# Allisterh/CCMMshadowrateVAR-code

Hardware: AMD Instinct MI355X
Metric: Gibbs sweeps/sec (chains x vintages) N=20 p=12 (higher is better)
Workload: dtype f64

## Files before the change

### ccmmshadowratevar-code_amd/csrc/ccmm_lag.h

```cpp
#pragma once
#include <algorithm>

#include "ccmm_internal.h"

namespace ccmm {

struct LagSel {
  const double* dpool;
  const int* idx;
  const int* colmap;
  int ldd, rows, p;
  int mode;
};
constexpr int kLagGramExport = 8;
constexpr int kLagNoSyrk = 1, kLagNoChol = 2;
constexpr int kLagNoFactorInv = 256;
constexpr int kLagNoTrailing = 1024;
constexpr int kLagNoV = 16, kLagNoXtv = 32, kLagNoSubst = 64, kLagNoXx = 128;

struct SolveXch {
  double* part;
  unsigned long long* flag;
  unsigned long long epoch;
};
constexpr int kSolveSplitMaxB = 64;

constexpr int kGlWaves = 8;
constexpr int kGlLd = 17;
constexpr int kGlTile = 16 * kGlLd;

__host__ __device__ constexpr int gl_ntile(int NT) { return NT * (NT + 1) / 2; }
__host__ __device__ constexpr int gl_tpw(int NT) { return (gl_ntile(NT) + kGlWaves - 1) / kGlWaves; }
__host__ __device__ constexpr int gl_tile(int NT, int i, int j) { return j * NT - j * (j - 1) / 2 + (i - j); }
__host__ __device__ constexpr int gl_tj(int NT, int g) {
  int tj = 0;
  while (tj < NT && g >= NT - tj) {
    g -= NT - tj;
    ++tj;
  }
  return tj;
}
__host__ __device__ constexpr int gl_ti(int NT, int g) {
  int tj = 0;
  while (tj < NT && g >= NT - tj) {
    g -= NT - tj;
    ++tj;
  }
  return tj + g;
}
__host__ __device__ constexpr int gl_out_len(int NT) { return gl_ntile(NT) * 256 + 256; }
inline size_t gl_lds_bytes(int NT, int rows, int ldd, int TP) {
  const size_t syrk = (size_t)rows * ldd + TP + 4;
  const size_t fac = 16 * NT + 8 + 64 + 2 * kGlTile + 2 * (size_t)NT * kGlTile + kGlWaves * kGlTile;
  return std::max(syrk, fac) * sizeof(double);
}

constexpr int kSlThreads = 512;

__host__ __device__ inline int sl_union(int NT, int TP) { return TP + 512; }
inline size_t sl_lds_bytes(int NT, int rows, int ldd, int TP, int nmax) {
  const size_t n = (size_t)rows * ldd + sl_union(NT, TP) + 256 + 256 + (size_t)nmax * nmax + 16;
  return n * sizeof(double) + (16 * NT + 32) * sizeof(int);
}

bool lag_supported_nt(int nt);
hipError_t lag_launch_gram(int NT, hipStream_t st, size_t lds, Dims d, const int* Tslot, LagSel ls,
                           ChainState cs, const double* iVdiag);
int lag_solve_resident(int NT, int nmax, size_t lds, int async);
hipError_t lag_launch_solve(int NT, int nmax, int async, hipStream_t st, size_t lds, Dims d, const int* Tslot,
                            const double* iVb, XSel xs, LagSel ls, ChainState cs, RngArgs ra, SolveXch xc);

}
```

### ccmmshadowratevar-code_amd/csrc/ccmm_lag.hip

```cpp
#include "ccmm_lag.h"

#include <cstdlib>

namespace ccmm {

struct GlArgs {
  const double* w;
  const double* iv;
  const int* colmap;
  double* out;
  int T, ldd, mode;
  const double* Dl;
  const double* swl;
};

__device__ __forceinline__ int gl_opaque(int v) {
  asm volatile("" : "+v"(v));
  return v;
}

__device__ __forceinline__ double gl_rsqrt_det(double d) { return rsqrt_det(d); }

__device__ __forceinline__ int gl_factor_inv(const double* Dg, double* Ws, int lane_in) {
  const int lane = gl_opaque(lane_in);
  double row[16];
  double rdiag = 1.0, dmin = 1.0;
#pragma unroll
  for (int m = 0; m < 16; ++m) row[m] = (lane < 16 && m <= lane) ? Dg[lane * kGlLd + m] : 0.0;
#pragma unroll
  for (int kk = 0; kk < 16; ++kk) {
    double dkk = readlane_d(row[kk], kk);
    dmin = fmin(dmin, dkk);
    const double rp = gl_rsqrt_det(fmax(dkk, 1e-300));
    if (lane == kk) rdiag = rp;
    const double lik = (lane > kk) ? row[kk] * rp : 0.0;
    row[kk] = lik;
#pragma unroll
    for (int m = kk + 1; m < 16; ++m) row[m] = fma(-lik, readlane_d(lik, m), row[m]);
  }
  const int bad = (dmin > 0.0) ? 0 : 1;
  const int c = lane;
  double x[16];
#pragma unroll
  for (int i = 0; i < 16; ++i) {
    double s0 = (i == c) ? 1.0 : 0.0, s1 = 0.0;
#pragma unroll
    for (int m = 0; m < i; m += 2) {
      s0 = fma(-readlane_d(row[m], i), x[m], s0);
      if (m + 1 < i) s1 = fma(-readlane_d(row[m + 1], i), x[m + 1], s1);
    }
    x[i] = (i >= c) ? (s0 + s1) * readlane_d(rdiag, i) : 0.0;
  }
  if (lane < 16) {
#pragma unroll
    for (int i = 0; i < 16; ++i) Ws[i * kGlLd + c] = x[i];
  }
  wave_lds_sync();
  return bad;
}

template <int NT, int W>
__device__ __forceinline__ void gl_syrk(const GlArgs& g, dbl4 (&acc)[gl_tpw(NT)], double& bs0, double& bs1,
                                        double& csum, int lane) {
  constexpr int NTILE = gl_ntile(NT);
  constexpr int TPW = gl_tpw(NT);
  const int lr = lane & 15, lq = lane >> 4;
#pragma unroll
  for (int k = 0; k < TPW; ++k) acc[k] = dbl4{0.0, 0.0, 0.0, 0.0};

  int off[NT];
#pragma unroll
  for (int b = 0; b < NT; ++b) off[b] = g.colmap[16 * b + lr];
  bs0 = 0.0;
  bs1 = 0.0;
  csum = 0.0;
  const int nks = (g.mode & kLagNoSyrk) ? 0 : (g.T + 3) >> 2;
  double raw[NT], sw = 0.0;
  auto load = [&](int ks) {
    const int t = 4 * ks + lq;
    sw = g.swl[t];
    const double* row = g.Dl + t * g.ldd;
#pragma unroll
    for (int b = 0; b < NT; ++b) raw[b] = row[off[b]];
  };
  if (nks > 0) load(0);
  for (int ks = 0; ks < nks; ++ks) {
    double frag[NT];
#pragma unroll
    for (int b = 0; b < NT; ++b) frag[b] = raw[b] * sw;
    const double swc = sw;
    load(ks + 1 < nks ? ks + 1 : ks);
    __builtin_amdgcn_sched_barrier(0);
#pragma unroll
    for (int k = 0; k < TPW; ++k) {
      if (W + kGlWaves * k < NTILE) {
        const int gi = W + kGlWaves * k;
        acc[k] = __builtin_amdgcn_mfma_f64_16x16x4f64(frag[gl_tj(NT, gi)], frag[gl_ti(NT, gi)], acc[k],
                                                      0, 0, 0);
      }
    }
    if (W < NT) bs0 = fma(frag[W < NT ? W : 0], swc, bs0);
    if (W + kGlWaves < NT) bs1 = fma(frag[W + kGlWaves < NT ? W + kGlWaves : 0], swc, bs1);
    csum = fma(swc, swc, csum);
    __builtin_amdgcn_sched_barrier(0);
  }
  bs0 += __shfl_xor(bs0, 16);
  bs0 += __shfl_xor(bs0, 32);
  bs1 += __shfl_xor(bs1, 16);
  bs1 += __shfl_xor(bs1, 32);
  csum += __shfl_xor(csum, 16);
  csum += __shfl_xor(csum, 32);
}

template <int NT>
__device__ __forceinline__ int gram_lag_factor(const GlArgs& g, double* sm, int tid, int W,
                                               dbl4 (&acc)[gl_tpw(NT)], double bs0, double bs1, double csum) {
  constexpr int NTILE = gl_ntile(NT);
  constexpr int TPW = gl_tpw(NT);
  constexpr int KL = 16 * NT;
  const int lane = tid & 63, lr0 = lane & 15, lq0 = lane >> 4;
  const int lr = lr0, lq = lq0;
  int bad = 0;
  int sti[TPW], stj[TPW];
#pragma unroll
  for (int k = 0; k < TPW; ++k) {
    const int gi = W + kGlWaves * k;
    sti[k] = gi < NTILE ? gl_ti(NT, gi) : 0;
    stj[k] = gi < NTILE ? gl_tj(NT, gi) : 0;
  }
  if (g.mode & kLagGramExport) {
    double* o = g.out;
#pragma unroll
    for (int k = 0; k < TPW; ++k) {
      const int gi = W + kGlWaves * k;
      if (gi < NTILE) {
#pragma unroll
        for (int r = 0; r < 4; ++r) o[gi * 256 + 64 * r + lane] = acc[k][r];
      }
    }
    if (lq == 0) {
      if (W < NT) o[NTILE * 256 + 1 + 16 * W + lr] = bs0;
      if (W + kGlWaves < NT) o[NTILE * 256 + 1 + 16 * (W + kGlWaves) + lr] = bs1;
    }
    if (W == 0 && lane == 0) o[NTILE * 256] = csum;
    return 0;
  }
  __syncthreads();

  double* lvec = sm;
  double* misc = lvec + KL;
  double* Dg = misc + 8;
  double* Pn0 = Dg + kGlTile;
  double* Ws = Pn0 + 2 * NT * kGlTile + W * kGlTile;

  if (lq == 0) {
    if (W < NT) lvec[16 * W + lr] = bs0;
    if (W + kGlWaves < NT) lvec[16 * (W + kGlWaves) + lr] = bs1;
  }
  if (W == 0 && lane == 0) misc[0] = csum;
  __syncthreads();
  const double G00 = misc[0] + g.iv[0];
  if (!(G00 > 0.0)) bad = 1;
  const double L00 = sqrt(G00 > 0.0 ? G00 : 1.0);
  const double rL00 = 1.0 / L00;
#pragma unroll
  for (int k = 0; k < TPW; ++k) {
    const int gi = W + kGlWaves * k;
    if (gi < NTILE) {
      const int ti = sti[k], tj = stj[k];
      const double lc = lvec[16 * ti + lr] * rL00;
#pragma unroll
      for (int r = 0; r < 4; ++r) {
        const int rowi = 16 * tj + lq + 4 * r;
        double v = fma(-(lvec[rowi] * rL00), lc, acc[k][r]);
        if (ti == tj && lq + 4 * r == lr) v += g.iv[1 + rowi];
        acc[k][r] = v;
      }
    }
  }
  __syncthreads();
  if (tid < KL) lvec[tid] *= rL00;
  __syncthreads();

  double* LinvB = Dg;
  const bool do_chol = !(g.mode & kLagNoChol);
  if (do_chol) {
    bool own = false;
#pragma unroll
    for (int k = 0; k < TPW; ++k) {
      const int gi = W + kGlWaves * k;
      if (gi < NTILE && sti[k] == 0 && stj[k] == 0) {
#pragma unroll
        for (int r = 0; r < 4; ++r) Ws[(lq + 4 * r) * kGlLd + lr] = acc[k][r];
        own = true;
      }
    }
    wave_lds_sync();
    if (own && !(g.mode & kLagNoFactorInv)) bad |= gl_factor_inv(Ws, LinvB, lane);
  }
  for (int p = 0; p < (do_chol ? NT : 0); ++p) {
    const int lr = gl_opaque(lr0), lq = gl_opaque(lq0);
    __syncthreads();
    double* Pn = Pn0;
#pragma unroll
    for (int k = 0; k < TPW; ++k) {
      const int gi = W + kGlWaves * k;
      if (gi < NTILE && stj[k] == p) {
        const int ti = sti[k];
        if (ti == p) {
#pragma unroll
          for (int r = 0; r < 4; ++r) acc[k][r] = LinvB[lr * kGlLd + lq + 4 * r];
        } else {
          dbl4 cc = dbl4{0.0, 0.0, 0.0, 0.0};
#pragma unroll
          for (int kk = 0; kk < 4; ++kk)
            cc = __builtin_amdgcn_mfma_f64_16x16x4f64(LinvB[lr * kGlLd + 4 * kk + lq], acc[k][kk], cc, 0, 0, 0);
#pragma unroll
          for (int r = 0; r < 4; ++r) Pn[ti * kGlTile + (lq + 4 * r) * kGlLd + lr] = cc[r];
          dbl4 mm = dbl4{0.0, 0.0, 0.0, 0.0};
#pragma unroll
          for (int kk = 0; kk < 4; ++kk)
            mm = __builtin_amdgcn_mfma_f64_16x16x4f64(LinvB[(4 * kk + lq) * kGlLd + lr], cc[kk], mm, 0, 0, 0);
          acc[k] = mm;
        }
      }
    }
    __syncthreads();
    if (p + 1 < NT && !(g.mode & kLagNoTrailing)) {
      const int q = p + 1;
      bool own = false;
#pragma unroll
      for (int k = 0; k < TPW; ++k) {
        const int gi = W + kGlWaves * k;
        if (gi < NTILE && sti[k] == q && stj[k] == q) {
#pragma unroll
          for (int kk = 0; kk < 4; ++kk) {
            const double pq = Pn[q * kGlTile + (4 * kk + lq) * kGlLd + lr];
            acc[k] = __builtin_amdgcn_mfma_f64_16x16x4f64(-pq, pq, acc[k], 0, 0, 0);
          }
#pragma unroll
          for (int r = 0; r < 4; ++r) Ws[(lq + 4 * r) * kGlLd + lr] = acc[k][r];
          own = true;
        }
      }
      wave_lds_sync();
      if (own && !(g.mode & kLagNoFactorInv)) bad |= gl_factor_inv(Ws, LinvB, lane);
#pragma unroll
      for (int k = 0; k < TPW; ++k) {
        const int gi = W + kGlWaves * k;
        if (gi < NTILE && stj[k] > p && !(sti[k] == q && stj[k] == q)) {
          const double* Pa = Pn + stj[k] * kGlTile + lq * kGlLd + lr;
          const double* Pb = Pn + sti[k] * kGlTile + lq * kGlLd + lr;
#pragma unroll
          for (int kk = 0; kk < 4; ++kk)
            acc[k] = __builtin_amdgcn_mfma_f64_16x16x4f64(-Pa[4 * kk * kGlLd], Pb[4 * kk * kGlLd], acc[k], 0, 0,
                                                          0);
        }
      }
    }
  }

  double* o = g.out;
  if (tid < KL) o[NTILE * 256 + 1 + tid] = lvec[tid];
  if (tid == 0) o[NTILE * 256] = rL00;
#pragma unroll
  for (int k = 0; k < TPW; ++k) {
    const int gi = W + kGlWaves * k;
    if (gi < NTILE) {
#pragma unroll
      for (int r = 0; r < 4; ++r) o[gi * 256 + 64 * r + lane] = acc[k][r];
    }
  }
  return bad;
}

template <int NT>
__global__ __launch_bounds__(512, 1) void k_gram_chol_lag(Dims d, const int* __restrict__ Tslot, LagSel ls,
                                                          ChainState cs, const double* __restrict__ iVdiag) {
  extern __shared__ double sm[];
  const int mat = blockIdx.x;
  const int c = mat / d.N, j = mat % d.N;
  const int s = cs.slot[c];
  const int tid = threadIdx.x;
  const int TP = d.TP;
  {
    const double* src = ls.dpool + (size_t)ls.idx[mat] * ls.rows * ls.ldd;
    const int n = ls.rows * ls.ldd;
    const double* w = cs.W + (size_t)mat * TP;
    double* swl = sm + n;
    int q = tid;
    for (; q < n; q += 32 * 512) {
      double v[32];
#pragma unroll
      for (int u = 0; u < 32; ++u) v[u] = (q + 512 * u < n) ? src[q + 512 * u] : 0.0;
      double wv[2];
#pragma unroll
      for (int u = 0; u < 2; ++u) wv[u] = (q == tid && tid + 512 * u < TP) ? w[tid + 512 * u] : 0.0;
#pragma unroll
      for (int u = 0; u < 32; ++u)
        if (q + 512 * u < n) sm[q + 512 * u] = v[u];
      if (q == tid) {
#pragma unroll
        for (int u = 0; u < 2; ++u)
          if (tid + 512 * u < TP + 4) swl[tid + 512 * u] = wv[u];
      }
    }
    for (int t = tid + 1024; t < TP + 4; t += 512) swl[t] = (t < TP) ? w[t] : 0.0;
  }
  __syncthreads();
  GlArgs g;
  g.T = Tslot[s];
  g.ldd = ls.ldd;
  g.mode = ls.mode;
  g.colmap = ls.colmap;
  g.iv = iVdiag + ((size_t)s * d.N + j) * d.KP;
  g.out = cs.G + (size_t)mat * d.KP * d.KP;
  g.Dl = sm;
  g.swl = sm + ls.rows * ls.ldd;
  g.w = nullptr;
  const int wave = __builtin_amdgcn_readfirstlane(tid >> 6);
  dbl4 acc[gl_tpw(NT)];
  double bs0, bs1, csum;
  switch (wave) {
    case 0: gl_syrk<NT, 0>(g, acc, bs0, bs1, csum, tid & 63); break;
    case 1: gl_syrk<NT, 1>(g, acc, bs0, bs1, csum, tid & 63); break;
    case 2: gl_syrk<NT, 2>(g, acc, bs0, bs1, csum, tid & 63); break;
    case 3: gl_syrk<NT, 3>(g, acc, bs0, bs1, csum, tid & 63); break;
    case 4: gl_syrk<NT, 4>(g, acc, bs0, bs1, csum, tid & 63); break;
    case 5: gl_syrk<NT, 5>(g, acc, bs0, bs1, csum, tid & 63); break;
    case 6: gl_syrk<NT, 6>(g, acc, bs0, bs1, csum, tid & 63); break;
    case 7: gl_syrk<NT, 7>(g, acc, bs0, bs1, csum, tid & 63); break;
    default: __builtin_unreachable();
  }
  const int bad = gram_lag_factor<NT>(g, sm, tid, wave, acc, bs0, bs1, csum);
  if (bad && (tid & 63) == 0) atomicOr(&cs.status[c], 2);
}

#ifdef CCMM_ABLATION
__device__ unsigned long long g_solve_prof[8];
extern "C" int ccmm_solve_prof(unsigned long long* out, int reset) {
  if (hipMemcpyFromSymbol(out, HIP_SYMBOL(g_solve_prof), sizeof(g_solve_prof)) != hipSuccess) return -1;
  if (reset) {
    static const unsigned long long z[8] = {};
    if (hipMemcpyToSymbol(HIP_SYMBOL(g_solve_prof), z, sizeof(z)) != hipSuccess) return -1;
  }
  return 0;
}
#define SL_CLK(x) const unsigned long long x = clock64()
#define SL_ACC(k, a, b) \
  if (c == 0 && blockIdx.y == 0 && tid == 0) atomicAdd(&g_solve_prof[k], (b) - (a))
#else
#define SL_CLK(x)
#define SL_ACC(k, a, b)
#endif
constexpr int kSlWaves = kSlThreads / 64;
template <int NT, int NMAX, bool RO>
__global__ __launch_bounds__(kSlThreads) void k_cta_solve_lag(Dims d, const int* __restrict__ Tslot,
                                                                const double* __restrict__ iVb, XSel xs, LagSel ls,
                                                                ChainState cs, RngArgs ra, SolveXch xc) {
  constexpr int NTILE = gl_ntile(NT);
  static_assert(kSlWaves == 8, "row-owned substitutions and the X'v t-halves: 8 waves");
  static_assert(!RO || NT == 1 || NT == 15, "row-owned substitutions: NT 1 or 15");
  constexpr int TPW = RO ? NT : (gl_ntile(NT) + kSlWaves - 1) / kSlWaves;
  constexpr int KL = 16 * NT;
  extern __shared__ double sm[];
  const int N = d.N, TP = d.TP, K = d.K, KP = d.KP;
  const int ldd = ls.ldd, rows = ls.rows;
  double* Dl = sm;
  double* vl = Dl + rows * ldd;
  double* part = vl + TP;
  double* rl = vl + sl_union(NT, TP);
  double* xl = rl + 256;
  double* Al = xl + 256;
  double* red = Al + NMAX * NMAX;
  int* cm = reinterpret_cast<int*>(red + 16);
  int* zdone = cm + KL;
  int* cnt = zdone + 16;
  const int c = blockIdx.x;
  const int s = cs.slot[c];
  const int T = Tslot[s];
  const int tid = threadIdx.x, lane0 = tid & 63;
  const int wave = __builtin_amdgcn_readfirstlane(tid >> 6);
  const Rng rng = ra.make(c);
  const bool split = gridDim.y > 1;
  const int hh = split ? (int)blockIdx.y : 0;
  const int th = (T + 1) >> 1;
  const int tlo = (split && hh) ? th : 0, thi = (split && !hh) ? th : TP;
  const double* ih2 = cs.ih2 + (size_t)c * N * TP;
  const double* Y = xs.ypool + (size_t)xs.yidx[c] * N * TP;
  double* E = cs.E + (size_t)c * N * TP;
  for (int q = tid; q < N * N; q += kSlThreads) Al[(q % N) + (q / N) * NMAX] = cs.A[(size_t)c * N * N + q];
  for (int q = tid; q < KL; q += kSlThreads) cm[q] = ls.colmap[q];
  int sti[TPW], stj[TPW];
  const int rHi = NT - 1 - wave, rLo = wave - 1;
  const bool hasHi = rHi >= 0, hasLo = wave >= 1 && rLo < rHi;
  const int nHi = hasHi ? rHi + 1 : 0, nLo = hasLo ? rLo + 1 : 0;
#pragma unroll
  for (int k = 0; k < TPW; ++k) {
    if constexpr (RO) {
      sti[k] = (k < nHi) ? rHi : rLo;
      stj[k] = (k < nHi) ? k : k - nHi;
    } else {
      const int gi = wave + kSlWaves * k;
      sti[k] = gi < NTILE ? gl_ti(NT, gi) : 0;
      stj[k] = gi < NTILE ? gl_tj(NT, gi) : 0;
    }
  }
  auto slot_of = [&](int k) -> int {
    if constexpr (RO) return (k < nHi + nLo) ? gl_tile(NT, sti[k], stj[k]) : -1;
    const int gi = wave + kSlWaves * k;
    return gi < NTILE ? gi : -1;
  };
  int cur = -1;

  for (int j = 0; j < N; ++j) {
    const int lane = gl_opaque(lane0), lr = lane & 15, lq = lane >> 4;
    const int mat = c * N + j;
    const int slab = ls.idx[mat];
    const double* Lo = cs.G + (size_t)mat * KP * KP;
    const double* Lv = Lo + NTILE * 256;
    if (slab != cur) {
      __syncthreads();
      const double* src = ls.dpool + (size_t)slab * rows * ldd;
      for (int q = tid; q < rows * ldd; q += 16 * kSlThreads) {
        double v[16];
#pragma unroll
        for (int u = 0; u < 16; ++u) v[u] = (q + kSlThreads * u < rows * ldd) ? src[q + kSlThreads * u] : 0.0;
#pragma unroll
        for (int u = 0; u < 16; ++u)
          if (q + kSlThreads * u < rows * ldd) Dl[q + kSlThreads * u] = v[u];
      }
      cur = slab;
    }
    SL_CLK(q0);
    for (int t = tlo + tid; t < thi; t += kSlThreads) {
      double acc = 0.0;
      if (t < T && !(ls.mode & kLagNoV)) {
        double e[NMAX];
        int o = t;
#pragma unroll
        for (int k = 0; k < NMAX; ++k) {
          if (k < N) e[k] = ((k == j) ? Y : E)[o];
          o += TP;
        }
        const double* wt = ih2 + t;
        double w0 = (j < N) ? wt[j * TP] : 0.0, w1 = (j + 1 < N) ? wt[(j + 1) * TP] : 0.0;
        double w2 = (j + 2 < N) ? wt[(j + 2) * TP] : 0.0, w3 = (j + 3 < N) ? wt[(j + 3) * TP] : 0.0;
#pragma unroll 1
        for (int i = j; i < N; ++i) {
          const double wi = w0;
          w0 = w1;
          w1 = w2;
          w2 = w3;
          w3 = (i + 4 < N) ? wt[(i + 4) * TP] : 0.0;
          const double* Ai = Al + i;
          double ea = 0.0;
#pragma unroll
          for (int k = 0; k < NMAX; ++k)
            if (k <= i) ea = fma(e[k], Ai[k * NMAX], ea);
          acc = fma(Ai[j * NMAX] * ea, wi, acc);
        }
      }
      vl[t] = acc;
    }
    __syncthreads();
    SL_CLK(q1);
    dbl4 lt[TPW];
#pragma unroll
    for (int k = 0; k < TPW; ++k) {
      const int gi = slot_of(k);
      if (gi >= 0) {
#pragma unroll
        for (int r = 0; r < 4; ++r) lt[k][r] = Lo[gi * 256 + 64 * r + lane];
      } else {
        lt[k] = dbl4{0.0, 0.0, 0.0, 0.0};
      }
    }
    const int nxv = split ? 256 : 512;
    {
      const int h = split ? hh : tid >> 8, a = tid & 255;
      const int t0 = h ? th : 0, t1 = h ? T : th;
      double p0 = 0.0, p1 = 0.0, p2 = 0.0, p3 = 0.0;
      if ((ls.mode & kLagNoXtv) || tid >= nxv) {
      } else if (a < KL) {
        const double* col = Dl + cm[a];
        int t = t0;
        for (; t + 7 < t1; t += 8) {
          double cv[8], vv[8];
#pragma unroll
          for (int u = 0; u < 8; ++u) {
            cv[u] = col[(t + u) * ldd];
            vv[u] = vl[t + u];
          }
          p0 = fma(cv[0], vv[0], p0);
          p1 = fma(cv[1], vv[1], p1);
          p2 = fma(cv[2], vv[2], p2);
          p3 = fma(cv[3], vv[3], p3);
          p0 = fma(cv[4], vv[4], p0);
          p1 = fma(cv[5], vv[5], p1);
          p2 = fma(cv[6], vv[6], p2);
          p3 = fma(cv[7], vv[7], p3);
        }
        if (t + 3 < t1) {
          p0 = fma(col[t * ldd], vl[t], p0);
          p1 = fma(col[(t + 1) * ldd], vl[t + 1], p1);
          p2 = fma(col[(t + 2) * ldd], vl[t + 2], p2);
          p3 = fma(col[(t + 3) * ldd], vl[t + 3], p3);
          t += 4;
        }
        for (; t < t1; ++t) p0 = fma(col[t * ldd], vl[t], p0);
      } else if (a == KL) {
        int t = t0;
        for (; t + 15 < t1; t += 16) {
          double vv[16];
#pragma unroll
          for (int u = 0; u < 16; ++u) vv[u] = vl[t + u];
#pragma unroll
          for (int u = 0; u < 16; ++u) p0 += vv[u];
        }
        for (; t < t1; ++t) p0 += vl[t];
      }
      if (tid < nxv) part[h * 256 + a] = (p0 + p1) + (p2 + p3);
    }
    __syncthreads();
    SL_CLK(q1b);
    SL_ACC(6, q1, q1b);
    if (split) {
      const int par = j & 1;
      double* mine = xc.part + (((size_t)c * 2 + hh) * 2 + par) * 256;
      const double* other = xc.part + (((size_t)c * 2 + (1 - hh)) * 2 + par) * 256;
      if (tid <= KL)
        __hip_atomic_store((unsigned long long*)(mine + tid), (unsigned long long)__double_as_longlong(part[hh * 256 + tid]),
                           __ATOMIC_RELAXED, __HIP_MEMORY_SCOPE_AGENT);
      asm volatile("s_waitcnt vmcnt(0)" ::: "memory");
      __syncthreads();
      const unsigned long long seq = xc.epoch * 64ull + (unsigned long long)j + 1ull;
      if (tid == 0) {
        __hip_atomic_store(&xc.flag[c * 2 + hh], seq, __ATOMIC_RELAXED, __HIP_MEMORY_SCOPE_AGENT);
        for (int it = 0;; ++it) {
          if (__hip_atomic_load(&xc.flag[c * 2 + 1 - hh], __ATOMIC_RELAXED, __HIP_MEMORY_SCOPE_AGENT) >= seq) break;
          if (it > (1 << 22)) {
            atomicOr(&cs.status[c], 32);
            break;
          }
          __builtin_amdgcn_s_sleep(2);
        }
      }
      __syncthreads();
      __builtin_amdgcn_fence(__ATOMIC_ACQUIRE, "wavefront");
      if (tid <= KL)
        part[(1 - hh) * 256 + tid] = __longlong_as_double((long long)__hip_atomic_load(
            (const unsigned long long*)(other + tid), __ATOMIC_RELAXED, __HIP_MEMORY_SCOPE_AGENT));
      __syncthreads();
    }
    SL_CLK(q2);
    const double* ivb = iVb + ((size_t)s * N + j) * KP;
    if (tid <= KL) {
      const int kx = (tid == KL) ? 0 : 1 + tid;
      rl[kx] = part[tid] + part[256 + tid] + ivb[kx];
    }
    __syncthreads();
    if (tid < KL) rl[1 + tid] = fma(-Lv[1 + tid], rl[0] * Lv[0], rl[1 + tid]);
    if (tid == KL) xl[0] = rl[0] * Lv[0];
    if (RO && tid < 16) {
      zdone[tid] = 0;
      cnt[tid] = 0;
    }
    __syncthreads();
    auto colsum = [&](const dbl4& t, const double* u) {
      double v = t[0] * u[0];
      v = fma(t[1], u[4], v);
      v = fma(t[2], u[8], v);
      v = fma(t[3], u[12], v);
      return xsum32(xsum16(v));
    };
    const bool subst = !(ls.mode & kLagNoSubst);
    bool stuck = false;
    auto wait_eq = [&](int* f, int v) {
      for (int it = 0; it < (1 << 22); ++it) {
        if (__hip_atomic_load(f, __ATOMIC_ACQUIRE, __HIP_MEMORY_SCOPE_WORKGROUP) == v) return;
        __builtin_amdgcn_s_sleep(1);
      }
      stuck = true;
    };
    auto post = [&](int* f, int v) {
      if (lane == 0) __hip_atomic_store(f, v, __ATOMIC_RELEASE, __HIP_MEMORY_SCOPE_WORKGROUP);
    };
    if constexpr (RO) {
      if (subst) {
#pragma unroll
        for (int h = 0; h < 2; ++h) {
          const bool has = h ? hasHi : hasLo;
          const int row = h ? rHi : rLo, k0 = h ? 0 : nHi;
          if (has) {
            double racc = rl[1 + 16 * row + lr];
#pragma unroll
            for (int k = 0; k < TPW; ++k) {
              if (k >= k0 && k <= k0 + row) {
                const int q = k - k0;
                if (q < row) {
                  wait_eq(zdone + q, 1);
                  racc -= colsum(lt[k], rl + 1 + 16 * q + lq);
                } else {
                  if (lq == 0) rl[1 + 16 * row + lr] = racc;
                  wave_lds_sync();
                  post(zdone + row, 1);
                  const double v = colsum(lt[k], rl + 1 + 16 * row + lq);
                  if (lq == 0) xl[1 + 16 * row + lr] = v;
                }
              }
            }
          }
        }
      }
    }
    for (int p = 0; p < ((subst && !RO) ? NT - 1 : 0); ++p) {
#pragma unroll
      for (int k = 0; k < TPW; ++k) {
        const int gi = wave + kSlWaves * k;
        if (gi < NTILE && stj[k] == p && sti[k] > p) {
          const double v = colsum(lt[k], rl + 1 + 16 * p + lq);
          if (lq == 0) rl[1 + 16 * sti[k] + lr] -= v;
        }
      }
      __syncthreads();
    }
    if (subst && !RO) {
#pragma unroll
      for (int k = 0; k < TPW; ++k) {
        const int gi = wave + kSlWaves * k;
        if (gi < NTILE && sti[k] == stj[k]) {
          const double v = colsum(lt[k], rl + 1 + 16 * sti[k] + lq);
          if (lq == 0) xl[1 + 16 * sti[k] + lr] = v;
        }
      }
    }
    __syncthreads();
    SL_CLK(q3);
    if (tid <= KL) {
      const int kx = (tid == KL) ? 0 : 1 + tid;
      rl[kx] = xl[kx] + ((kx < K) ? rng.normal(CCMM_RNG_PAI, (uint32_t)(kx + K * j)) : 0.0);
    }
    __syncthreads();
    {
      const bool b8 = lr & 8, b4 = lr & 4;
      auto fold = [&](const dbl4& t, double cv) {
        const double v0 = t[0] * cv, v1 = t[1] * cv, v2 = t[2] * cv, v3 = t[3] * cv;
        double a = b8 ? v2 : v0, b = b8 ? v3 : v1;
        a += dpp_d<0x128>(b8 ? v0 : v2);
        b += dpp_d<0x128>(b8 ? v1 : v3);
        double q = b4 ? b : a;
        const double x4 = b4 ? a : b;
        const double s4l = dpp_d<0x104>(x4), s4r = dpp_d<0x114>(x4);
        q += b4 ? s4r : s4l;
        q += dpp_d<0x4E>(q);
        q += dpp_d<0xB1>(q);
        return q;
      };
      if (subst) {
#pragma unroll
        for (int k = 0; k < TPW; ++k) {
          const bool diag = RO ? (slot_of(k) >= 0 && sti[k] == stj[k])
                               : (wave + kSlWaves * k < NTILE && sti[k] == stj[k]);
          if (diag) {
            const double q = fold(lt[k], rl[1 + 16 * sti[k] + lr]);
            if ((lr & 3) == 0) xl[1 + 16 * sti[k] + lq + 4 * (lr >> 2)] = q;
          }
        }
      }
      __syncthreads();
      if constexpr (RO) {
        if (subst) {
#pragma unroll
          for (int h = 1; h >= 0; --h) {
            const bool has = h ? hasHi : hasLo;
            const int row = h ? rHi : rLo, k0 = h ? 0 : nHi;
            if (has) {
              wait_eq(cnt + row, NT - 1 - row);
              const double xp = xl[1 + 16 * row + lr];
#pragma unroll
              for (int k = TPW - 1; k >= 0; --k) {
                if (k >= k0 && k < k0 + row) {
                  const int i = k - k0;
                  const double q = fold(lt[k], xp);
                  wait_eq(cnt + i, NT - 1 - row);
                  if ((lr & 3) == 0) xl[1 + 16 * i + lq + 4 * (lr >> 2)] -= q;
                  wave_lds_sync();
                  post(cnt + i, NT - row);
                }
              }
            }
          }
        }
        if (stuck && lane == 0) atomicOr(&cs.status[c], 32);
        __syncthreads();
      }
      for (int p = ((subst && !RO) ? NT - 1 : 0); p >= 1; --p) {
#pragma unroll
        for (int k = 0; k < TPW; ++k) {
          const int gi = wave + kSlWaves * k;
          if (gi < NTILE && sti[k] == p && stj[k] < p) {
            const double q = fold(lt[k], xl[1 + 16 * p + lr]);
            if ((lr & 3) == 0) xl[1 + 16 * stj[k] + lq + 4 * (lr >> 2)] -= q;
          }
        }
        __syncthreads();
      }
    }
    {
      double pr = (tid < KL) ? Lv[1 + tid] * xl[1 + tid] : 0.0;
      pr = wave_sum_dpp(pr);
      if (lane == 0) red[wave] = pr;
    }
    __syncthreads();
    if (tid == KL) {
      double sacc = 0.0;
      for (int w = 0; w < kSlThreads / 64; ++w) sacc += red[w];
      xl[0] = (rl[0] - sacc) * Lv[0];
    }
    __syncthreads();
    SL_CLK(q4);
    double* pai = cs.PAI + ((size_t)c * N + j) * KP;
    if (hh == 0)
      for (int k = tid; k < KP; k += kSlThreads) pai[k] = (k < K) ? xl[k] : 0.0;
    for (int t = tlo + tid; t < thi; t += kSlThreads) {
      double o = 0.0;
      if (t < T && !(ls.mode & kLagNoXx)) {
        const double* rowp = Dl + t * ldd;
        double s0 = xl[0], s1 = 0.0, s2 = 0.0, s3 = 0.0;
        if ((N & 3) == 0) {
          const int P = ls.p;
          for (int l = 1; l <= P; ++l) {
            const double* row = rowp + (P - l) * ldd;
            const double* xa = xl + 1 + (l - 1) * N;
#pragma unroll
            for (int k = 0; k < NMAX; k += 4) {
              if (k < N) {
                const double d0 = row[k], d1 = row[k + 1], d2 = row[k + 2], d3 = row[k + 3];
                s0 = fma(d0, xa[k], s0);
                s1 = fma(d1, xa[k + 1], s1);
                s2 = fma(d2, xa[k + 2], s2);
                s3 = fma(d3, xa[k + 3], s3);
              }
            }
          }
        } else {
          int a = 0;
          for (; a + 3 < KL; a += 4) {
            s0 = fma(rowp[cm[a]], xl[1 + a], s0);
            s1 = fma(rowp[cm[a + 1]], xl[2 + a], s1);
            s2 = fma(rowp[cm[a + 2]], xl[3 + a], s2);
            s3 = fma(rowp[cm[a + 3]], xl[4 + a], s3);
          }
          for (; a < KL; ++a) s0 = fma(rowp[cm[a]], xl[1 + a], s0);
        }
        o = Y[(size_t)j * TP + t] - ((s0 + s1) + (s2 + s3));
      }
      E[(size_t)j * TP + t] = o;
    }
    __syncthreads();
    SL_CLK(q5);
    SL_ACC(0, q0, q1);
    SL_ACC(1, q1, q2);
    SL_ACC(2, q2, q3);
    SL_ACC(3, q3, q4);
    SL_ACC(4, q4, q5);
    if (j == 0) SL_ACC(5, 0ull, 1ull);
  }
}


bool lag_supported_nt(int nt) { return nt == 1 || nt == 15; }

hipError_t lag_launch_gram(int NT, hipStream_t st, size_t lds, Dims d, const int* Tslot, LagSel ls,
                           ChainState cs, const double* iVdiag) {
  auto go = [&](auto k) { return launch_k(k, dim3(d.nmat), dim3(512), lds, true, st, d, Tslot, ls, cs, iVdiag); };
  switch (NT) {
    case 1: return go(k_gram_chol_lag<1>);
    case 15: return go(k_gram_chol_lag<15>);
    default: return hipErrorInvalidValue;
  }
}

constexpr int sl_key(int NT, int nmax) { return 100 * NT + nmax; }
template <class R, class F>
static R solve_instance(int NT, int nmax, bool ro, R none, F f) {
  switch (sl_key(NT, nmax)) {
    case sl_key(1, 8): return ro ? f(k_cta_solve_lag<1, 8, true>) : f(k_cta_solve_lag<1, 8, false>);
    case sl_key(1, 20): return ro ? f(k_cta_solve_lag<1, 20, true>) : f(k_cta_solve_lag<1, 20, false>);
    case sl_key(1, 32): return ro ? f(k_cta_solve_lag<1, 32, true>) : f(k_cta_solve_lag<1, 32, false>);
    case sl_key(15, 8): return ro ? f(k_cta_solve_lag<15, 8, true>) : f(k_cta_solve_lag<15, 8, false>);
    case sl_key(15, 20): return ro ? f(k_cta_solve_lag<15, 20, true>) : f(k_cta_solve_lag<15, 20, false>);
    case sl_key(15, 32): return ro ? f(k_cta_solve_lag<15, 32, true>) : f(k_cta_solve_lag<15, 32, false>);
    default: return none;
  }
}

int lag_solve_resident(int NT, int nmax, size_t lds, int async) {
  return solve_instance(NT, nmax, async != 0, 0, [&](auto k) {
    int per_cu = 0, dev = 0, cus = 0;
    if (raise_lds(k, lds) != hipSuccess) return 0;
    if (hipOccupancyMaxActiveBlocksPerMultiprocessor(&per_cu, (const void*)k, kSlThreads, lds) != hipSuccess) return 0;
    if (hipGetDevice(&dev) != hipSuccess ||
        hipDeviceGetAttribute(&cus, hipDeviceAttributeMultiprocessorCount, dev) != hipSuccess)
      return 0;
    return per_cu * cus;
  });
}

hipError_t lag_launch_solve(int NT, int nmax, int async, hipStream_t st, size_t lds, Dims d, const int* Tslot,
                            const double* iVb, XSel xs, LagSel ls, ChainState cs, RngArgs ra, SolveXch xc) {
  return solve_instance(NT, nmax, async != 0, hipErrorInvalidValue, [&](auto k) {
    return launch_k(k, dim3(d.B, xc.part ? 2 : 1), dim3(kSlThreads), lds, true, st, d, Tslot, iVb, xs, ls, cs, ra, xc);
  });
}

}
```

Before: 25480.

## Lookahead blocked Cholesky: defer trailing updates via double-buffered panels

Double-buffers the panel scratch (Pn alternates between two halves by step parity). The wave that owns the next diagonal tile applies its own update and factor-inverts it immediately, deferring its other trailing-tile updates to the next step using the previous panel buffer. It also raises wave priority during the trailing phase and adds ablation-only clock profiling. The aim is to take the diagonal factor-inverse off the critical path between barriers, at the cost of extra bookkeeping and more complex control flow.

```diff
diff --git a/ccmmshadowratevar-code_amd/csrc/ccmm_lag.h b/ccmmshadowratevar-code_amd/csrc/ccmm_lag.h
--- a/ccmmshadowratevar-code_amd/csrc/ccmm_lag.h
+++ b/ccmmshadowratevar-code_amd/csrc/ccmm_lag.h
@@ -49,10 +49,12 @@
   return tj + g;
 }
 __host__ __device__ constexpr int gl_out_len(int NT) { return gl_ntile(NT) * 256 + 256; }
+__host__ __device__ constexpr size_t gl_fac_doubles(int NT) {
+  return 16 * (size_t)NT + 8 + kGlTile + 2 * (size_t)NT * kGlTile + (size_t)kGlWaves * kGlTile;
+}
 inline size_t gl_lds_bytes(int NT, int rows, int ldd, int TP) {
   const size_t syrk = (size_t)rows * ldd + TP + 4;
-  const size_t fac = 16 * NT + 8 + 64 + 2 * kGlTile + 2 * (size_t)NT * kGlTile + kGlWaves * kGlTile;
-  return std::max(syrk, fac) * sizeof(double);
+  return std::max(syrk, gl_fac_doubles(NT)) * sizeof(double);
 }
 
 constexpr int kSlThreads = 512;
diff --git a/ccmmshadowratevar-code_amd/csrc/ccmm_lag.hip b/ccmmshadowratevar-code_amd/csrc/ccmm_lag.hip
--- a/ccmmshadowratevar-code_amd/csrc/ccmm_lag.hip
+++ b/ccmmshadowratevar-code_amd/csrc/ccmm_lag.hip
@@ -13,6 +13,25 @@
   const double* Dl;
   const double* swl;
 };
+
+#ifdef CCMM_ABLATION
+__device__ unsigned long long g_gram_prof[16];
+extern "C" int ccmm_gram_prof(unsigned long long* out, int reset) {
+  if (hipMemcpyFromSymbol(out, HIP_SYMBOL(g_gram_prof), sizeof(g_gram_prof)) != hipSuccess) return -1;
+  if (reset) {
+    static const unsigned long long z[16] = {};
+    if (hipMemcpyToSymbol(HIP_SYMBOL(g_gram_prof), z, sizeof(z)) != hipSuccess) return -1;
+  }
+  return 0;
+}
+#define GL_CLK(x) const unsigned long long x = clock64()
+#define GL_ACC(k, cond, a, b) \
+  if (blockIdx.x == 0 && (threadIdx.x & 63) == 0 && (cond)) atomicAdd(&g_gram_prof[k], (b) - (a))
+#define GL_OWNER(NT, t) (((t) * (NT) - (t) * ((t) - 1) / 2) % kGlWaves)
+#else
+#define GL_CLK(x)
+#define GL_ACC(k, cond, a, b)
+#endif
 
 __device__ __forceinline__ int gl_opaque(int v) {
   asm volatile("" : "+v"(v));
@@ -145,12 +164,13 @@
     if (W == 0 && lane == 0) o[NTILE * 256] = csum;
     return 0;
   }
+  GL_CLK(f0);
   __syncthreads();
 
   double* lvec = sm;
   double* misc = lvec + KL;
-  double* Dg = misc + 8;
-  double* Pn0 = Dg + kGlTile;
+  double* LinvB = misc + 8;
+  double* Pn0 = LinvB + kGlTile;
   double* Ws = Pn0 + 2 * NT * kGlTile + W * kGlTile;
 
   if (lq == 0) {
@@ -182,7 +202,9 @@
   if (tid < KL) lvec[tid] *= rL00;
   __syncthreads();
 
-  double* LinvB = Dg;
+  GL_CLK(f1);
+  GL_ACC(2, W == 0, f0, f1);
+
   const bool do_chol = !(g.mode & kLagNoChol);
   if (do_chol) {
     bool own = false;
@@ -197,11 +219,18 @@
     }
     wave_lds_sync();
     if (own && !(g.mode & kLagNoFactorInv)) bad |= gl_factor_inv(Ws, LinvB, lane);
-  }
+    GL_CLK(f2);
+    GL_ACC(6, own, f1, f2);
+  }
+  int pend = -1;
   for (int p = 0; p < (do_chol ? NT : 0); ++p) {
     const int lr = gl_opaque(lr0), lq = gl_opaque(lq0);
-    __syncthreads();
-    double* Pn = Pn0;
+    const int q = p + 1;
+    double* Pn = Pn0 + (p & 1) * NT * kGlTile;
+    const double* Po = Pn0 + (q & 1) * NT * kGlTile;
+    GL_CLK(c0);
+    __syncthreads();
+    GL_CLK(c1);
 #pragma unroll
     for (int k = 0; k < TPW; ++k) {
       const int gi = W + kGlWaves * k;
@@ -225,14 +254,24 @@
         }
       }
     }
-    __syncthreads();
-    if (p + 1 < NT && !(g.mode & kLagNoTrailing)) {
-      const int q = p + 1;
-      bool own = false;
+    GL_CLK(c2);
+    __syncthreads();
+    GL_CLK(c3);
+    const bool trail = q < NT && !(g.mode & kLagNoTrailing);
+    bool own = false;
+    if (trail) {
 #pragma unroll
       for (int k = 0; k < TPW; ++k) {
         const int gi = W + kGlWaves * k;
         if (gi < NTILE && sti[k] == q && stj[k] == q) {
+          __builtin_amdgcn_s_setprio(3);
+          if (pend >= 0) {
+#pragma unroll
+            for (int kk = 0; kk < 4; ++kk) {
+              const double pq = Po[q * kGlTile + (4 * kk + lq) * kGlLd + lr];
+              acc[k] = __builtin_amdgcn_mfma_f64_16x16x4f64(-pq, pq, acc[k], 0, 0, 0);
+            }
+          }
 #pragma unroll
           for (int kk = 0; kk < 4; ++kk) {
             const double pq = Pn[q * kGlTile + (4 * kk + lq) * kGlLd + lr];
@@ -245,21 +284,47 @@
       }
       wave_lds_sync();
       if (own && !(g.mode & kLagNoFactorInv)) bad |= gl_factor_inv(Ws, LinvB, lane);
+    }
+    GL_CLK(c4);
+    if (trail) {
 #pragma unroll
       for (int k = 0; k < TPW; ++k) {
         const int gi = W + kGlWaves * k;
         if (gi < NTILE && stj[k] > p && !(sti[k] == q && stj[k] == q)) {
-          const double* Pa = Pn + stj[k] * kGlTile + lq * kGlLd + lr;
-          const double* Pb = Pn + sti[k] * kGlTile + lq * kGlLd + lr;
-#pragma unroll
-          for (int kk = 0; kk < 4; ++kk)
-            acc[k] = __builtin_amdgcn_mfma_f64_16x16x4f64(-Pa[4 * kk * kGlLd], Pb[4 * kk * kGlLd], acc[k], 0, 0,
-                                                          0);
-        }
-      }
-    }
-  }
-
+          const int oa = stj[k] * kGlTile + lq * kGlLd + lr, ob = sti[k] * kGlTile + lq * kGlLd + lr;
+          if (pend >= 0) {
+#pragma unroll
+            for (int kk = 0; kk < 4; ++kk)
+              acc[k] = __builtin_amdgcn_mfma_f64_16x16x4f64(-Po[oa + 4 * kk * kGlLd], Po[ob + 4 * kk * kGlLd], acc[k],
+                                                            0, 0, 0);
+          }
+          if (!own || stj[k] == q) {
+#pragma unroll
+            for (int kk = 0; kk < 4; ++kk)
+              acc[k] = __builtin_amdgcn_mfma_f64_16x16x4f64(-Pn[oa + 4 * kk * kGlLd], Pn[ob + 4 * kk * kGlLd], acc[k],
+                                                            0, 0, 0);
+          }
+        }
+      }
+      pend = (own && q + 1 < NT) ? p : -1;
+      __builtin_amdgcn_s_setprio(0);
+    }
+    GL_CLK(c5);
+#ifdef CCMM_ABLATION
+    {
+      const int obs = (q < NT && GL_OWNER(NT, q) == 0) ? 1 : 0;
+      const int obs0 = (p > 0 && GL_OWNER(NT, p) == 0) ? 1 : 0;
+      GL_ACC(3, W == obs0, c0, c1);
+      GL_ACC(4, W == obs, c1, c2);
+      GL_ACC(5, W == obs, c2, c3);
+      GL_ACC(6, own, c3, c4);
+      GL_ACC(7, own, c4, c5);
+      GL_ACC(8, W == obs && trail, c3, c5);
+    }
+#endif
+  }
+
+  GL_CLK(f3);
   double* o = g.out;
   if (tid < KL) o[NTILE * 256 + 1 + tid] = lvec[tid];
   if (tid == 0) o[NTILE * 256] = rL00;
@@ -271,6 +336,8 @@
       for (int r = 0; r < 4; ++r) o[gi * 256 + 64 * r + lane] = acc[k][r];
     }
   }
+  GL_CLK(f4);
+  GL_ACC(9, W == 0, f3, f4);
   return bad;
 }
 
@@ -283,6 +350,7 @@
   const int s = cs.slot[c];
   const int tid = threadIdx.x;
   const int TP = d.TP;
+  GL_CLK(k0);
   {
     const double* src = ls.dpool + (size_t)ls.idx[mat] * ls.rows * ls.ldd;
     const int n = ls.rows * ls.ldd;
@@ -308,6 +376,7 @@
     for (int t = tid + 1024; t < TP + 4; t += 512) swl[t] = (t < TP) ? w[t] : 0.0;
   }
   __syncthreads();
+  GL_CLK(k1);
   GlArgs g;
   g.T = Tslot[s];
   g.ldd = ls.ldd;
@@ -332,8 +401,14 @@
     case 7: gl_syrk<NT, 7>(g, acc, bs0, bs1, csum, tid & 63); break;
     default: __builtin_unreachable();
   }
+  GL_CLK(k2);
   const int bad = gram_lag_factor<NT>(g, sm, tid, wave, acc, bs0, bs1, csum);
   if (bad && (tid & 63) == 0) atomicOr(&cs.status[c], 2);
+  GL_CLK(k3);
+  GL_ACC(0, wave == 0, k0, k1);
+  GL_ACC(1, wave == 0, k1, k2);
+  GL_ACC(10, wave == 0, 0ull, 1ull);
+  GL_ACC(11, wave == 0, k0, k3);
 }
 
 #ifdef CCMM_ABLATION
```

Measured after the change: 25600 (median of 6 runs). Within noise of the previous version (+0.5%).
